# mcbuehler/Seg2Eye

Measured on AMD Instinct MI355X. Metric: images/sec per G+D train step, 256x256 bs=8, higher is better.
Workload: dtype bf16; 1 GPU; Seg2Eye G+D hinge-GAN train step (G step + D step, TTUR Adam, GAN + GAN_Feat), 256x256, batch 8 per GPU, ngf=ndf=64, 4 style images, synthetic ellipse labels, 4 batches in rotation; global_batch=8, parallelism=dp1, gradient_exchange=none, graph_segments_G=1

## Files before the change

### include/seg2eye_hip.h

```cpp
#ifndef SEG2EYE_HIP_H
#define SEG2EYE_HIP_H
#include <stddef.h>
#include <stdint.h>

#ifdef __cplusplus
extern "C" {
#endif

#define S2E_OK 0
#define S2E_ERR_ARG (-1)
#define S2E_ERR_LAUNCH (-2)
#define S2E_ERR_UNSUPPORTED (-3)

enum { S2E_F32 = 0, S2E_BF16 = 1 };
enum { S2E_ACT_NONE = 0, S2E_ACT_LRELU = 1, S2E_ACT_TANH = 2 };
enum { S2E_AUX_NONE = 0, S2E_AUX_RELU_MASK = 1, S2E_AUX_LRELU_GRAD = 2 };
enum { S2E_NORM_SPADE_STYLE = 0, S2E_NORM_PLAIN_IN = 1,
       S2E_NORM_SPADE_STYLE_BATCH = 2,
       S2E_NORM_ACCUMULATE_DX = 0x100 };
enum { S2E_LOSS_NEG_MEAN = 0, S2E_LOSS_HINGE_REAL = 1, S2E_LOSS_HINGE_FAKE = 2, S2E_LOSS_L1 = 3,
       S2E_LOSS_L1_NANGRAD = 4 };

int s2e_version(void);
const char* s2e_last_error(void);
// ... 126 lines not shown
    const int* rect_list; const int* rect_count;
    int N, H, W, Cin, Cout;
    int flags;
} s2e_wgrad_batch_job;
int s2e_wgrad_batch_supported(int dtype, int N, int H, int W, int Cin, int Cout);
size_t s2e_wgrad_batch_workspace_bytes(void);
int s2e_wgrad_batch(int dtype, const s2e_wgrad_batch_job* jobs, int n_jobs, void* workspace, size_t workspace_bytes, void* stream);
int s2e_spade_conv_modulate_rect(int dtype, int N, int H, int W, int C, int nh, int flags, int* tw, int* th);
#define S2E_UNI_REPLICAS 16
typedef struct s2e_spade_uni_job {
    const float* R; float* A; const float* w_gb; long w_sc, w_sk, w_st;
    const float* w_sh; const float* b_sh; float* dw_sh; float* db_sh; float* dw_gb; float* db_gb;
    int C2, nh, ncls, act_bf16;
} s2e_spade_uni_job;
int s2e_label_rect_lists_bwd(const uint8_t* cls, int N, int tiles_y, int tiles_x, int* work_list, int* ui_list, int* counts, void* stream);
int s2e_conv2d_rects_supported(int dtype, const s2e_conv_desc* d);
int s2e_conv2d_rects(int dtype, const void* x, const void* w_packed, const float* bias, const void* residual, const void* aux, void* y,
                     const s2e_conv_desc* d, const int* rect_list, const int* rect_count, void* stream);
size_t s2e_conv2d_wgrad_rects_workspace_bytes(int dtype, const s2e_conv_desc* d);
int s2e_conv2d_wgrad_rects(int dtype, const void* x, const void* gy, float* dw, float* dbias, const s2e_conv_desc* d,
                           const int* rect_list, const int* rect_count, void* workspace, size_t workspace_bytes, void* stream);
int s2e_spade_uniform_sums(int dtype, const void* dgb, int N, int H, int W, int C2, int ncls, const uint8_t* cls, const int* ui_list,
                           const int* counts, float* R, void* stream);
int s2e_spade_uniform_grads(const s2e_spade_uni_job* jobs_host, int n_jobs, void* stream);
int s2e_label_rect_classify(const uint8_t* label, int N, int H, int W, int h, int w, int tw, int th,
                            uint8_t* cls, int* dense_list, int* uni_list, int* counts, void* stream);
int s2e_spade_conv_modulate_sparse(int dtype, const void* actv, const void* w_packed, const float* bias, const void* x,
                                   const float* stats, const float* style, int style_ld, void* out, void* gamma_out,
                                   int N, int H, int W, int C, int nh, int lrelu, int flags, const int* dense_list,
                                   const int* counts, void* stream);
// ... 166 lines not shown
```

### seg2eye_amd/_lib.py

```python
import ctypes as C
import os

import torch

_HERE = os.path.dirname(os.path.abspath(__file__))
LIB_PATH = os.environ.get('S2E_LIB_PATH') or os.path.join(_HERE, 'lib', 'libseg2eye_hip.so')

S2E_F32, S2E_BF16 = 0, 1
UNI_REPLICAS = 16
SPADE_ANY_TILES, SPADE_DENSE, SPADE_ANY_RECTS, SPADE_X_HALF = 1, 2, 4, 8
ACT_NONE, ACT_LRELU, ACT_TANH = 0, 1, 2
AUX_NONE, AUX_RELU_MASK, AUX_LRELU_GRAD = 0, 1, 2
NORM_SPADE_STYLE, NORM_PLAIN_IN, NORM_SPADE_STYLE_BATCH = 0, 1, 2
NORM_ACCUMULATE_DX = 0x100
LOSS_NEG_MEAN, LOSS_HINGE_REAL, LOSS_HINGE_FAKE, LOSS_L1, LOSS_L1_NANGRAD = 0, 1, 2, 3, 4
REGION_L1, REGION_L2 = 0, 1
RANK_L2, RANK_MISMATCH = 0, 1


class ConvDesc(C.Structure):
    _fields_ = [(n, C.c_int) for n in (
        'N', 'Hi', 'Wi', 'Cin', 'Ho', 'Wo', 'Cout', 'KH', 'KW', 'stride', 'pad',
        'transposed', 'in_act', 'out_act', 'aux_mode')]

# ... 69 lines not shown
    's2e_weight_grads_batched': (STATUS, [_vp, _vp, _i, _i, _i, _vp, _vp]),
    's2e_unpack_weight_grad': (STATUS, [_vp, _vp, _i, _i, _i, _i, _i, _i, _vp]),
    's2e_pack_block_map': (COUNT, [_i, _vp, _i, _vp]),
    's2e_pack_conv_weights': (STATUS, [_i, _vp, _vp, _i, _i, _vp, _vp]),
    's2e_conv2d_workspace_bytes': (SIZE, [_i, C.POINTER(ConvDesc)]),
    's2e_conv2d_kernel_kind': (VALUE, [_i, C.POINTER(ConvDesc)]),
    's2e_conv2d_wgrad_kernel_kind': (VALUE, [_i, C.POINTER(ConvDesc)]),
    's2e_conv2d': (STATUS, [_i, _vp, _vp, _vp, _vp, _vp, _vp, C.POINTER(ConvDesc), _vp, C.c_size_t, _vp]),
    's2e_conv2d_plane_supported': (VALUE, [_i, C.POINTER(ConvDesc)]),
    's2e_conv_plane_weight_elems': (SIZE, [C.POINTER(ConvDesc)]),
    's2e_conv2d_plane': (STATUS, [_i, _vp, _vp, _vp, _vp, _vp, _vp, C.POINTER(ConvDesc), _vp]),
    's2e_conv2d_stats_slots': (VALUE, [_i, C.POINTER(ConvDesc)]),
    's2e_conv2d_stats': (STATUS, [_i, _vp, _vp, _vp, _vp, _vp, C.POINTER(ConvDesc), _vp, _vp]),
    's2e_in_stats_from_partials': (STATUS, [_vp, _i, _i, _i, _i, _f, _vp, _vp, _vp]),
    's2e_label_rect_lists_bwd': (STATUS, [_vp, _i, _i, _i, _vp, _vp, _vp, _vp]),
    's2e_conv2d_rects_supported': (VALUE, [_i, C.POINTER(ConvDesc)]),
    's2e_conv2d_rects': (STATUS, [_i, _vp, _vp, _vp, _vp, _vp, _vp, C.POINTER(ConvDesc), _vp, _vp, _vp]),
    's2e_conv2d_wgrad_rects_workspace_bytes': (SIZE, [_i, C.POINTER(ConvDesc)]),
    's2e_conv2d_wgrad_rects': (STATUS, [_i, _vp, _vp, _vp, _vp, C.POINTER(ConvDesc), _vp, _vp, _vp, C.c_size_t, _vp]),
    's2e_spade_uniform_sums': (STATUS, [_i, _vp, _i, _i, _i, _i, _i, _vp, _vp, _vp, _vp, _vp]),
    's2e_spade_uniform_grads': (STATUS, [_vp, _i, _vp]),
    's2e_conv2d_wgrad_workspace_bytes': (SIZE, [_i, C.POINTER(ConvDesc)]),
    's2e_conv2d_wgrad': (STATUS, [_i, _vp, _vp, _vp, _vp, C.POINTER(ConvDesc), _vp, C.c_size_t, _vp]),
    's2e_conv2d_wgrad_multi_supported': (VALUE, [_i, C.POINTER(ConvDesc)]),
    's2e_conv2d_wgrad_multi_kind': (VALUE, [_i, C.POINTER(ConvDesc)]),
    's2e_conv2d_wgrad_multi_workspace_bytes': (SIZE, [_i, _vp, _i]),
    's2e_conv2d_wgrad_multi': (STATUS, [_i, _vp, _i, _vp, C.c_size_t, _vp]),
    's2e_in_stats_workspace_bytes': (SIZE, [_i, _i, _i, _i]),
    's2e_modulate_bwd_workspace_bytes': (SIZE, [_i, _i, _i, _i]),
    's2e_instance_norm_fwd': (STATUS, [_i, _vp, _vp, _vp, _vp, _i, _i, _i, _f, _i, _vp]),
# ... 156 lines not shown
```

### seg2eye_amd/csrc/conv_duo.hip

```cpp
#include "conv_patch.h"
#include <stdlib.h>

namespace {

struct DuoParams {
    const void* x; const void* w; const float* bias; const void* res; const void* aux; void* y;
    int N, Hi, Wi, Cin, Ho, Wo, Cout, Kpad;
    int org, flip, out_act, aux_mode;
    int tw, th, sh, tw_shift;
    int tiles_x, tiles_y, tiles_n;
    int rects;
    unsigned x_bytes, w_bytes;
    const int* rect_list; const int* rect_count;
    const void* mx; const float* mstats; const float* mstyle; int msld; void* mgamma; int mC, mlrelu, mup;
    float* spart; int sP;
    long* dbg;
    int abl;
};

constexpr int DU_PPX = 400;
constexpr int DU_P_BYTES = DU_PPX * 64;
constexpr int DU_B_BYTES = 128 * 64;
constexpr int DU_NBS = 3, DU_PD = 2;

template <bool FUSE, int BN = 128, bool MF16 = false, int EPI = -1>
__global__ __launch_bounds__(256, 2) void conv_duo_kernel(const DuoParams p) {
    static_assert(BN == 128 || (BN == 64 && !FUSE), "tile widths");
    static_assert(!MF16 || BN == 128, "the 16x16x32 loop is written for 128-channel tiles");
    typedef bf16_t T;
    constexpr int NW = 4, TAPS = 9;
    constexpr int TM = BN / 32, TN = 2;
    constexpr int WROWS = TM * 32, NPASS = 2 * TM;
    constexpr int P_BYTES = DU_P_BYTES, B_BYTES = DU_B_BYTES, NBS = DU_NBS, PD = DU_PD;
    constexpr int NPIECE = P_BYTES / 1024;
    constexpr int NR = (NPIECE + NW - 1) / NW;
    constexpr int NBJ = BN / 64;
    constexpr int NR16 = 6;
    static_assert(NR <= TAPS, "one patch piece per tap must cover the patch");
    static_assert(NW * 4096 <= P_BYTES, "the waves' staging slices must fit one patch buffer");
    __shared__ __attribute__((aligned(16))) char smem[2 * P_BYTES + NBS * B_BYTES];
    __shared__ __attribute__((aligned(16))) float kcst[2][512];

// ... 160 lines not shown
        const int i = lane & 15, kq = lane >> 4;
#pragma unroll
        for (int dx = 0; dx < 3; ++dx)
            a16[dx] = lds0 + (uint32_t)(((8 * wm) * 18 + i + dx) * 64 + ((kq ^ (((i + dx) >> 1) & 3)) << 4));
        b16 = lds0 + 2 * P_BYTES + (uint32_t)((FUSE ? wn * 32 : wn * 64) * 64 + i * 64 + ((kq ^ ((i >> 1) & 3)) << 4));
    }
    auto read_al = [&](uint32_t ab, int dy) __attribute__((always_inline)) {
#pragma unroll
        for (int m = 0; m < 4; ++m)
            asm volatile("ds_read_b128 %0, %1 offset:%2" : "=v"(fal[m]) : "v"(ab), "n"((m + dy) * 1152) : "memory");
    };
    auto read_ah = [&](uint32_t ab, int dy) __attribute__((always_inline)) {
#pragma unroll
        for (int m = 0; m < 4; ++m)
            asm volatile("ds_read_b128 %0, %1 offset:%2" : "=v"(fah[m]) : "v"(ab), "n"((4 + m + dy) * 1152) : "memory");
    };
    auto read_b = [&](uint32_t bb, int par) __attribute__((always_inline)) {
#pragma unroll
        for (int n = 0; n < 4; ++n)
            asm volatile("ds_read_b128 %0, %1 offset:%2" : "=v"(fbb[par][n]) : "v"(bb), "n"(FUSE ? (n & 1) * 1024 + (n >> 1) * 4096 : n * 1024) : "memory");
    };
    auto mfma16 = [&](int half, int par) __attribute__((always_inline)) {
#pragma unroll
        for (int m = 0; m < 4; ++m)
#pragma unroll
            for (int n = 0; n < 4; ++n)
                acc16[MF16 ? half * 4 + m : 0][n] = __builtin_amdgcn_mfma_f32_16x16x32_bf16(
                    __builtin_bit_cast(bf16x8_t, half ? fah[m] : fal[m]), __builtin_bit_cast(bf16x8_t, fbb[par][n]), acc16[MF16 ? half * 4 + m : 0][n], 0, 0, 0);
    };

// ... 208 lines not shown
                }
            });
            *(u32x4_t*)(yg + so + lo) = u32x4_t{ov[0], ov[1], ov[2], ov[3]};
            if (gout) *(u32x4_t*)(gout + so + lo) = u32x4_t{gv[0], gv[1], gv[2], gv[3]};
        });
        st_issued = gout ? 16 : 8;
    };

    auto fetch_rect = [&](int id) __attribute__((always_inline)) -> int {
        if (p.rect_list && id < n_items) return p.rect_list[id / p.tiles_n];
        return -1;
    };

    Item cur = decode(item_id, fetch_rect(item_id));
    aim(cur);
    int pb = 0, cb = 0;
    prologue(cur, pb, cb);
    int tile_i = (int)blockIdx.x >= (G >> 1) ? 1 : 0;
#ifdef S2E_DUO_STAMPS
    int dbg_i = 0;
    const bool dbg_on = p.dbg && tid == 0 && ((int)blockIdx.x == 0 || (int)blockIdx.x == (G >> 1) || (int)blockIdx.x == 8);
    long* dbg_row = p.dbg ? p.dbg + ((int)blockIdx.x == 0 ? 0 : (int)blockIdx.x == 8 ? 2 : 1) * 64 : nullptr;
    auto stamp = [&](int k) __attribute__((always_inline)) { if (dbg_on && dbg_i < 12) dbg_row[dbg_i * 5 + k] = __builtin_amdgcn_s_memrealtime(); };
#else
    auto stamp = [&](int) __attribute__((always_inline)) {};
#endif
    for (;;) {
        stamp(0);
        if (st_issued >= 16) wait_vmcnt<16>();
        else if (st_issued >= 8) wait_vmcnt<8>();
// ... 43 lines not shown
                static_for<0, 2 * TAPS>([&](auto T) {
                    constexpr int t = decltype(T)::value;
                    constexpr int tap = t % TAPS, cc = t / TAPS, par = t & 1;
                    constexpr int ntap = (tap + 1) % TAPS, u = t + PD;
                    uint32_t pcb = cc ? pbs1 : pbs0, pnb = cc ? pbs0 : pbs1;
                    uint32_t nsb = (uint32_t)(((t + 1) % NBS) * B_BYTES);
                    int cs = c;
                    asm volatile("" : "+s"(pcb), "+s"(pnb), "+s"(nsb), "+s"(cs));
                    if (cs >= nch) return;
#ifdef S2E_DUO_STAMPS
                    const int abl = p.abl;
#else
                    constexpr int abl = 0;
#endif
                    if (!(abl & 1)) {
                        if constexpr (tap < NR16) { if (cc == 0 || !last) dma_patch16(tap, cs + cc + 1, pnb); }
                        if (u < 2 * TAPS || !last) dma_w16(cs + u / TAPS, u % TAPS, u % NBS);
                    }
                    if (!(abl & 4)) read_ah(a16[tap % 3] + pcb, tap / 3);
                    asm volatile("s_waitcnt lgkmcnt(4)" : "+v"(fal[0]), "+v"(fal[1]), "+v"(fal[2]), "+v"(fal[3]), "+v"(fbb[par][0]), "+v"(fbb[par][1]),
                                 "+v"(fbb[par][2]), "+v"(fbb[par][3]) :: "memory");
                    if (!(abl & 2)) mfma16(0, par);
                    constexpr int now_p = tap < NR16 ? 1 : 0, now_w = NBJ;
                    if constexpr (cc == 1 && (tap < NR16 || u >= 2 * TAPS)) {
                        if (last) wait_keep(u < 2 * TAPS ? now_w : 0); else wait_keep(now_p + now_w);
                    } else wait_keep(now_p + now_w);
                    asm volatile("s_waitcnt lgkmcnt(0)" : "+v"(fah[0]), "+v"(fah[1]), "+v"(fah[2]), "+v"(fah[3]) :: "memory");
                    if (!(abl & 8)) __builtin_amdgcn_s_barrier();
                    if (!(abl & 4)) {
                        if (t + 1 < 2 * TAPS || !last) {
                            read_al(a16[ntap % 3] + (ntap == 0 ? pnb : pcb), ntap / 3);
                            read_b(b16 + nsb, par ^ 1);
                        }
                    }
                    if (!(abl & 2)) mfma16(1, par);
                });
            }
        } else {
        float cinit[TN];
            {
// ... 12 lines not shown
            for (int mi = 0; mi < TM; ++mi)
    #pragma unroll
                for (int ni = 0; ni < TN; ++ni)
    #pragma unroll
                    for (int r = 0; r < 16; ++r) acc[mi][ni][r] = cinit[ni];
            int kt = 0, stage = 0;
            aim_frags(0, 0, pb, 0);
            read_frags(0, 0);
            for (int c = 0; c < nch; ++c) {
                const bool more = c + 1 < nch;
                const int pcur = (pb + c) & 1;
                static_for<0, TAPS>([&](auto TAP) {
                    constexpr int tap = decltype(TAP)::value;
                    constexpr int ntap = (tap + 1) % TAPS;
                    int issued = 0;
                    if constexpr (tap < NR) { if (more) issued += dma_patch(TAP, c + 1, pcur ^ 1); }
                    if (kt + PD < nk) { dma_w(kt + PD, stage == 0 ? NBS - 1 : stage - 1); issued += NBJ; }
                    read_frags(1, 1);
                    frags_ready(0, false);
                    mfmas(0);
                    wait_keep(issued);
                    frags_ready(1, true);
                    __builtin_amdgcn_s_barrier();
                    stage = stage == NBS - 1 ? 0 : stage + 1;
                    ++kt;
                    if (kt < nk) {
                        aim_frags(ntap / 3, ntap % 3, ntap == 0 ? pcur ^ 1 : pcur, stage);
                        read_frags(0, 0);
                    }
                    mfmas(1);
                });
            }
        }
        stamp(2);
        __builtin_amdgcn_s_setprio(0);
        const int pbn = (pb + nch) & 1;
        const int next_id = item_id + G;
        const bool has_next = next_id < n_items;
        Item nxt = cur;
        if constexpr (FUSE) load_mod_consts(cb);
        if (has_next) { nxt = decode(next_id, nf); aim(nxt); prologue(nxt, pbn, cb ^ 1); }
        stamp(3);
        if constexpr (FUSE) epilogue_fused(cur, pbn ^ 1);
        else if constexpr (EPI == 0) epilogue(cur, pbn ^ 1, std::integral_constant<int, 0>{}, std::false_type{});
        else if constexpr (EPI == 1) epilogue(cur, pbn ^ 1, std::integral_constant<int, 1>{}, std::false_type{});
        else if constexpr (EPI == 2) epilogue(cur, pbn ^ 1, std::integral_constant<int, 2>{}, std::false_type{});
// ... 8 lines not shown
        else epilogue(cur, pbn ^ 1, std::integral_constant<int, 0>{}, std::false_type{});
        stamp(4);
#ifdef S2E_DUO_STAMPS
        ++dbg_i;
#endif
        if (!has_next) break;
        cur = nxt; item_id = next_id; pb = pbn; cb ^= 1; ++tile_i;
    }
}

int duo_min_items() {
    static const int n = s2e_env_int("S2E_CONV_DUO", 256);
    return n;
}

template <bool FUSE>
int duo_launch(DuoParams& p, long rects_upper, hipStream_t st) {
    const long items = rects_upper * p.tiles_n;
    const int cap = 2 * s2e_cu_count();
    const int grid = items < cap ? (int)items : cap;
#ifdef S2E_DUO_STAMPS
    static long* const dbg_ptr = (long*)s2e_env_long("S2E_DUO_DBG_PTR", 0);
    p.dbg = dbg_ptr;
    static const int abl_env = s2e_env_int("S2E_DUO_ABL", 0);
    p.abl = abl_env;
#endif
    static const bool mf16 = s2e_env_flag("S2E_DUO_MF16", true);
    if (!FUSE && p.Cout <= 64) conv_duo_kernel<false, 64><<<grid, 256, 0, st>>>(p);
    else if (!mf16) conv_duo_kernel<FUSE><<<grid, 256, 0, st>>>(p);
    else if (FUSE) conv_duo_kernel<true, 128, true><<<grid, 256, 0, st>>>(p);
    else {
        const int epi = p.aux_mode != S2E_AUX_NONE ? 2 : (p.res ? 1 : 0) + (p.spart ? 3 : 0);
        if (epi == 0) conv_duo_kernel<false, 128, true, 0><<<grid, 256, 0, st>>>(p);
        else if (epi == 1) conv_duo_kernel<false, 128, true, 1><<<grid, 256, 0, st>>>(p);
        else if (epi == 2) conv_duo_kernel<false, 128, true, 2><<<grid, 256, 0, st>>>(p);
        else if (epi == 3) conv_duo_kernel<false, 128, true, 3><<<grid, 256, 0, st>>>(p);
        else conv_duo_kernel<false, 128, true, 4><<<grid, 256, 0, st>>>(p);
    }
    S2E_CHECK_LAUNCH("conv_duo_kernel");
    return S2E_OK;
}

}
// ... 36 lines not shown
int s2e_conv_duo_stats_slots(const s2e_conv_desc* d, const s2e_patch_plan* plan) {
    return (d->Ho / plan->th) * (d->Wo / plan->tw) * (d->Cout <= 64 ? 4 : 2);
}

int s2e_conv_duo_launch(const s2e_patch_plan* plan, const void* x, const void* w, const float* bias, const void* res,
                        const void* aux, void* y, const s2e_conv_desc* d, int kpad, float* stats_part, const int* rect_list,
                        const int* rect_count, hipStream_t st) {
    DuoParams p{};
    p.x = x; p.w = w; p.bias = bias; p.res = res; p.aux = aux; p.y = y;
    p.rect_list = rect_list; p.rect_count = rect_count;
    p.spart = stats_part; p.sP = stats_part ? s2e_conv_duo_stats_slots(d, plan) : 0;
    duo_fill(&p, d, plan, kpad);
    p.tiles_n = d->Cout <= 64 ? 1 : ceil_div(d->Cout, 128);
    p.w_bytes = (unsigned)((long)s2e_conv_cout_pad(d->Cout) * kpad * 2);
    return duo_launch<false>(p, p.rects, st);
}

int s2e_spade_conv_modulate_duo(int dtype, const void* actv, const void* w_packed, const float* bias, const void* x,
                                const float* stats, const float* style, int style_ld, void* out, void* gamma_out,
                                int N, int H, int W, int C, int nh, int lrelu, int flags, int tw, int th,
                                const int* rect_list, const int* rect_count, hipStream_t st) {
    if (duo_min_items() <= 0 || dtype != S2E_BF16 || nh % 32 != 0 || C % 64 != 0 || (flags & S2E_SPADE_ANY_TILES)) return 0;
    if (!duo_rect_ok(tw, th, H, W)) return 0;
    const long rects = (long)N * (H / th) * (W / tw);
    if (rects * (C / 64) < duo_min_items()) return 0;
    if ((long)N * H * W * nh * 2 >= (1L << 31) || (long)N * H * W * C * 2 >= (1L << 31)) return 0;
    const int kpad = ceil_div(9 * nh, 64) * 64;
    if ((long)s2e_conv_cout_pad(2 * C) * kpad * 2 >= (1L << 31)) return 0;
    const s2e_conv_desc d{N, H, W, nh, H, W, 2 * C, 3, 3, 1, 1, 0, S2E_ACT_NONE, S2E_ACT_NONE, S2E_AUX_NONE};
    const s2e_patch_plan plan{tw, th, 1, 0, 0};
// ... 12 lines not shown
```

### seg2eye_amd/csrc/conv_igemm.hip

```cpp
#include "common.h"
#include "conv_small.h"
#include "conv_patch.h"
#include "conv_stream.h"
#include <stdlib.h>

struct ConvKParams {
    const void* x; const void* w; const float* bias; const void* res; const void* aux; void* y;
    int N, Hi, Wi, Cin, Ho, Wo, Cout;
    int KH, KW, stride, pad, transposed;
    int in_act, out_act, aux_mode;
    int Ktot, Kpad, M, tiles_n;
    int tm_fast;
    int tiles, splits, kt_per_split;
    float* partial;
    int cls_tile0[5];
};


template <typename T, int BN, bool VECPATH, bool GLDS, bool S2 = false>
__global__ __launch_bounds__(256, 2) void conv_igemm_kernel(const ConvKParams p) {
    constexpr int BM = 128;
    constexpr int VEC = Vec<T>::N;
    constexpr int BK = 8 * VEC;
    constexpr int WN = (BN >= 64) ? 2 : 1;
// ... 550 lines not shown
extern "C" int s2e_conv2d_rects_supported(int dtype, const s2e_conv_desc* d) {
    return d && conv_route(dtype, d, false).kernel == ROUTE_DUO ? 1 : 0;
}

extern "C" int s2e_conv2d_rects(int dtype, const void* x, const void* w, const float* bias, const void* res, const void* aux, void* y,
                                const s2e_conv_desc* d, const int* rect_list, const int* rect_count, void* stream) {
    if (!x || !w || !y || !d || !rect_list || !rect_count) S2E_FAIL(S2E_ERR_ARG, "s2e_conv2d_rects: null pointer");
    if (d->aux_mode != S2E_AUX_NONE && !aux) S2E_FAIL(S2E_ERR_ARG, "s2e_conv2d_rects: aux_mode without aux");
    const ConvRoute r = conv_route(dtype, d, res && d->aux_mode != S2E_AUX_NONE);
    if (r.kernel != ROUTE_DUO)
        S2E_FAIL(S2E_ERR_UNSUPPORTED, "s2e_conv2d_rects: this shape's kernel takes no rectangle list (s2e_conv2d_rects_supported)");
    return s2e_conv_duo_launch(&r.patch, x, w, bias, res, aux, y, d, s2e_conv_k_pad(dtype, d->KH * d->KW * d->Cin), nullptr, rect_list, rect_count,
                               (hipStream_t)stream);
}

extern "C" int s2e_conv2d(int dtype, const void* x, const void* w, const float* bias, const void* res,
                          const void* aux, void* y, const s2e_conv_desc* d, void* workspace, size_t workspace_bytes,
                          void* stream) {
    if (!x || !w || !y || !d) S2E_FAIL(S2E_ERR_ARG, "s2e_conv2d: null pointer");
    if (d->stride != 1 && d->stride != 2) S2E_FAIL(S2E_ERR_UNSUPPORTED, "s2e_conv2d: stride %d", d->stride);
    if (d->N <= 0 || d->Cin <= 0 || d->Cout <= 0 || d->Ho <= 0 || d->Wo <= 0 || d->Hi <= 0 || d->Wi <= 0)
        S2E_FAIL(S2E_ERR_ARG, "s2e_conv2d: bad shape");
    if (d->aux_mode != S2E_AUX_NONE && !aux) S2E_FAIL(S2E_ERR_ARG, "s2e_conv2d: aux_mode without aux");
    if (d->KH * d->KW > 32) S2E_FAIL(S2E_ERR_UNSUPPORTED, "s2e_conv2d: kernel %dx%d has more than 32 taps", d->KH, d->KW);
    if ((long)d->N * d->Hi * d->Wi >= (1L << 31) || (long)d->N * d->Ho * d->Wo >= (1L << 31))
        S2E_FAIL(S2E_ERR_UNSUPPORTED, "s2e_conv2d: tensor too large for 32-bit pixel indices");
    const ConvRoute r = conv_route(dtype, d, res && d->aux_mode != S2E_AUX_NONE);
    if (r.workspace_bytes && (!workspace || workspace_bytes < r.workspace_bytes))
        S2E_FAIL(S2E_ERR_ARG, "s2e_conv2d: this shape needs %zu bytes of workspace (s2e_conv2d_workspace_bytes)", r.workspace_bytes);
    hipStream_t st = (hipStream_t)stream;
// ... 40 lines not shown
```

### seg2eye_amd/csrc/conv_patch.h

```cpp
#pragma once
#include "common.h"

struct s2e_patch_plan {
    int tw, th;
    int splits;
    int s2d;
    int bn;
};
int s2e_conv_patch_plan(int dtype, const s2e_conv_desc* d, s2e_patch_plan* plan);
int s2e_conv_patch_launch(int dtype, const s2e_patch_plan* plan, const void* x, const void* w, const float* bias, const void* res,
                          const void* aux, void* y, const s2e_conv_desc* d, int kpad, float* partial, hipStream_t st);

double s2e_patch_rectangle(const s2e_conv_desc* d, int ks, int* tw_out, int* th_out);

int s2e_conv_duo_plan(int dtype, const s2e_conv_desc* d, s2e_patch_plan* plan);
int s2e_conv_duo_launch(const s2e_patch_plan* plan, const void* x, const void* w, const float* bias, const void* res,
                        const void* aux, void* y, const s2e_conv_desc* d, int kpad, float* stats_part, const int* rect_list,
                        const int* rect_count, hipStream_t st);
int s2e_conv_duo_stats_slots(const s2e_conv_desc* d, const s2e_patch_plan* plan);
int s2e_spade_conv_modulate_duo(int dtype, const void* actv, const void* w_packed, const float* bias, const void* x,
                                const float* stats, const float* style, int style_ld, void* out, void* gamma_out,
                                int N, int H, int W, int C, int nh, int lrelu, int flags, int tw, int th,
                                const int* rect_list, const int* rect_count, hipStream_t st);
```

### seg2eye_amd/networks/architecture.py

```python
import torch
import torch.nn as nn
from torch.nn.utils import spectral_norm

from .. import ops
from ..spectral import sn_begin
from .normalization import SPADE_STYLE_Block, SegMap, spade_stats


class SPADE_STYLE_ResnetBlock(nn.Module):

    def __init__(self, fin, fout, opt):
        super().__init__()
        fmid = min(fin, fout)
        self.learned_shortcut = fin != fout
        wrap = spectral_norm if 'spectral' in opt.norm_G else (lambda conv: conv)
        convs = [('conv_0', fin, fmid, 3, True), ('conv_1', fmid, fout, 3, True)]
        norms = [('norm_0', fin), ('norm_1', fmid)]
        if self.learned_shortcut:
            convs.append(('conv_s', fin, fout, 1, False))
            norms.append(('norm_s', fin))
        for name, cin, cout, k, bias in convs:
            setattr(self, name, wrap(nn.Conv2d(cin, cout, kernel_size=k, padding=k // 2, bias=bias)))
        for name, c in norms:
            setattr(self, name, SPADE_STYLE_Block(c, opt))

    def input_stats(self, x, replication=1):
        ready = getattr(x, '_s2e_in_stats', None)
        if ready is not None and self.norm_0.spade.kind == 'instance':
            return ready
        return spade_stats(x, [self.norm_0.spade] + ([self.norm_s.spade] if self.learned_shortcut else []), replication)

    def _convs(self, h0, x_s, seg, latent_style):
        fused = self.norm_1.spade.kind == 'instance'
        s_dx, s_out = ([], []) if fused else (None, None)
        dx = ops.conv2d_m(h0, self.conv_0, None, 1, 1, stats_out=s_dx)
        out = ops.conv2d_m(self.norm_1(dx, seg, latent_style, s_dx[0] if s_dx else None, lrelu=True), self.conv_1, x_s, 1, 1, stats_out=s_out)
        if s_out:
            out._s2e_in_stats = s_out[0]
        return out

    def forward(self, x, seg, latent_style, stats=None, up=False):
        seg = SegMap.of(seg)
        sn_begin(self)
        fold = (up and self.learned_shortcut and stats is not None and self.norm_0.spade.kind != 'batch'
                and self.norm_0.takes_fold(x) and self.norm_s.takes_fold(x))
        if up and not fold:
            x = ops.upsample2x(x)
        if fold:
            if torch.is_grad_enabled() and x.requires_grad:
                h0, x = self.norm_0(x, seg, latent_style, stats, lrelu=True, relay=True, up=True)
            else:
                h0 = self.norm_0(x, seg, latent_style, stats, lrelu=True, up=True)
            x_s = ops.conv2d_m(self.norm_s(x, seg, latent_style, stats, lrelu=False, up=True), self.conv_s)
            return self._convs(h0, x_s, seg, latent_style)
        if stats is None:
            stats = self.input_stats(x)
        if torch.is_grad_enabled() and x.requires_grad:
            h0, x = self.norm_0(x, seg, latent_style, stats, lrelu=True, relay=True)
        else:
            h0 = self.norm_0(x, seg, latent_style, stats, lrelu=True)
        if self.learned_shortcut:
            x_s = ops.conv2d_m(self.norm_s(x, seg, latent_style, stats, lrelu=False), self.conv_s)
        else:
            x_s = x
        return self._convs(h0, x_s, seg, latent_style)
```

### seg2eye_amd/networks/generator.py

```python
import os

import torch
import torch.nn as nn

from .. import ops
from .._lib import ACT_LRELU, ACT_TANH
from ..options import latent_size
from .. import packing
from . import stylebank
from ..spectral import sn_begin
from .architecture import SPADE_STYLE_ResnetBlock
from .base_network import BaseNetwork, compute_dtype_of
from .normalization import SegMap


_FOLD_UP = os.environ.get('S2E_FOLD_UPSAMPLE', '1') != '0'


class SPADESTYLEGenerator(BaseNetwork):
    @staticmethod
    def modify_commandline_options(parser, is_train):
        parser.add_argument('--num_upsampling_layers', choices=('normal', 'more'), default='normal',
                            help="If 'more', adds upsampling layer between the two middle resnet blocks "
                                 "('most' is broken in the reference and not offered)")
# ... 1 lines not shown

    def __init__(self, opt):
        super().__init__()
        self.opt = opt
        self.cdtype = compute_dtype_of(opt)
        nf = opt.ngf
        self.sw, self.sh = latent_size(opt)
        self.fc = nn.Conv2d(opt.semantic_nc, 16 * nf, 3, padding=1)
        self.head_0 = SPADE_STYLE_ResnetBlock(16 * nf, 16 * nf, opt)
        self.G_middle_0 = SPADE_STYLE_ResnetBlock(16 * nf, 16 * nf, opt)
        self.G_middle_1 = SPADE_STYLE_ResnetBlock(16 * nf, 16 * nf, opt)
        self.up_0 = SPADE_STYLE_ResnetBlock(16 * nf, 8 * nf, opt)
        self.up_1 = SPADE_STYLE_ResnetBlock(8 * nf, 4 * nf, opt)
        self.up_2 = SPADE_STYLE_ResnetBlock(4 * nf, 2 * nf, opt)
        self.up_3 = SPADE_STYLE_ResnetBlock(2 * nf, 1 * nf, opt)
        self.conv_img = nn.Conv2d(nf, opt.output_nc, 3, padding=1)
        self.up = nn.Upsample(scale_factor=2)

    def forward(self, input, w=None):
        seg = SegMap.of(input)
        self.require_gpu(seg.label, w)
        n, H, W = seg.shape
        f = 32 if self.opt.num_upsampling_layers == 'normal' else 64
        if (H, W) != (self.sh * f, self.sw * f):
            raise ValueError('label map is %dx%d but this generator emits %dx%d (SURVEY F5)' % (H, W, self.sh * f, self.sw * f))
        w = w.float()
        bank = sn_begin(self)
        pre = self.__dict__.get('_spade_prepass')
        if pre is None:
            pre = self.__dict__['_spade_prepass'] = ops.SpadePrepass()
# ... 27 lines not shown
```

### seg2eye_amd/ops/conv.py

```python
import collections

import torch

from .. import _lib as L
from .. import packing
from .._lib import ConvDesc, ACT_NONE, ACT_LRELU, ACT_TANH, AUX_NONE, AUX_LRELU_GRAD
from .core import IN_EPS, LaunchProfiler, ZeroPool, _cl_dense, _cl_rows, _dt, _grad_dst, _need, _p, _stream, colsum, memo
from .sink import GradSink



PLANE_LAYOUT = 4


def pack_weight(w_oihw, dtype, cin_pad=None, transposed=False, sigma=None, plane=False):
    dt = _dt(dtype)
    w = w_oihw.detach()
    cout, cin, kh, kw = w.shape
    cin_pad = cin if cin_pad is None else cin_pad
    if plane:
        if dtype != torch.bfloat16 or cin_pad != cin:
            raise ValueError('pack_weight: the plane layout is bf16 without channel padding')
        cl = w.dtype == torch.float32 and not w.is_contiguous() and _cl_dense(w)
        if not cl and (w.dtype != torch.float32 or not w.is_contiguous()):
# ... 285 lines not shown
            gres = g
        return gx, gw, gb, gres, None, None, None, None, None, None, None, None


def conv2d(x, weight, bias=None, residual=None, stride=1, pad=0, in_act=ACT_NONE, out_act=ACT_NONE, sn=None, stats_out=None):
    u, v, sigma = sn if sn is not None else (None, None, None)
    return Conv2dFn.apply(x, weight, bias, residual, stride, pad, in_act, out_act, u, v, sigma, stats_out)


def conv2d_m(x, conv, residual=None, stride=1, pad=0, in_act=ACT_NONE, out_act=ACT_NONE, stats_out=None):
    from ..spectral import conv_params
    weight, bias, sn = conv_params(conv)
    return conv2d(x, weight, bias, residual, stride, pad, in_act, out_act, sn, stats_out)


class FcHeadFn(torch.autograd.Function):

    @staticmethod
    def forward(ctx, x, weight, bias, slope):
        _need(x, weight, bias)
        m, h, w, c = x.shape
        n = weight.shape[0]
        y = torch.empty(m, n, dtype=torch.float32, device=x.device)
        wsb = L.call.s2e_fc_head_fwd_workspace_bytes(m, h * w, c, n)
        ws = torch.empty(max(wsb // 4, 1), dtype=torch.float32, device=x.device)
        L.call.s2e_fc_head_fwd(_dt(x), _p(x), _p(weight), _p(bias), _p(y), m, h * w, c, n, float(slope), _p(ws), wsb, _stream())
        ctx.slope = float(slope)
        ctx.wdst, ctx.bdst = _grad_dst(weight), _grad_dst(bias)
        ctx.save_for_backward(x, weight)
        return y
# ... 21 lines not shown
```

### seg2eye_amd/ops/switches.py

```python
import os

_DET = os.environ.get('S2E_DETERMINISTIC', '0') == '1'

WGRAD_BATCH_OFF = os.environ.get('S2E_WGRAD_BATCH', '1') == '0' or _DET
WGRAD_MULTI_OFF = os.environ.get('S2E_WGRAD_MULTI', '1') == '0'
SPARSE_BWD_OFF = os.environ.get('S2E_SPADE_SPARSE_BWD', '1') == '0' or _DET
SPARSE_OFF = os.environ.get('S2E_SPADE_SPARSE', '1') == '0'
FUSED_OFF = os.environ.get('S2E_SPADE_FUSED', '1') == '0'
C8_SPARSE_OFF = os.environ.get('S2E_C8_SPARSE', '1') == '0'
```

Measured before the change: 539.5 images/s.

## Fold learned 1x1 shortcut conv into the 3x3 conv_1 duo kernel as extra K chunks

Adds a FOLD variant of the duo implicit-GEMM kernel that, after the 3x3 conv_1 accumulation, streams the shortcut activations and 1x1 weights through the patch and weight buffers as an extra K tail. The shortcut conv is then computed into the same accumulators instead of being materialised as a residual tensor. This is wired into the up_1..up_3 resnet blocks through a new autograd function whose backward calls the two existing conv backward paths. It saves one launch and the write and re-read of x_s per block, at the cost of more kernel template variants and a longer per-tile K loop.

```diff
diff --git a/include/seg2eye_hip.h b/include/seg2eye_hip.h
--- a/include/seg2eye_hip.h
+++ b/include/seg2eye_hip.h
@@ -164,6 +164,9 @@
     int C2, nh, ncls, act_bf16;
 } s2e_spade_uni_job;
 int s2e_label_rect_lists_bwd(const uint8_t* cls, int N, int tiles_y, int tiles_x, int* work_list, int* ui_list, int* counts, void* stream);
+int s2e_conv2d_fold1x1_supported(int dtype, const s2e_conv_desc* d, int Cin2);
+int s2e_conv2d_fold1x1(int dtype, const void* x, const void* w_packed, const float* bias, const void* x2, const void* w2_packed, void* y,
+                       const s2e_conv_desc* d, int Cin2, float* stats_part, void* stream);
 int s2e_conv2d_rects_supported(int dtype, const s2e_conv_desc* d);
 int s2e_conv2d_rects(int dtype, const void* x, const void* w_packed, const float* bias, const void* residual, const void* aux, void* y,
                      const s2e_conv_desc* d, const int* rect_list, const int* rect_count, void* stream);
diff --git a/seg2eye_amd/_lib.py b/seg2eye_amd/_lib.py
--- a/seg2eye_amd/_lib.py
+++ b/seg2eye_amd/_lib.py
@@ -107,6 +107,8 @@
     's2e_conv2d_stats': (STATUS, [_i, _vp, _vp, _vp, _vp, _vp, C.POINTER(ConvDesc), _vp, _vp]),
     's2e_in_stats_from_partials': (STATUS, [_vp, _i, _i, _i, _i, _f, _vp, _vp, _vp]),
     's2e_label_rect_lists_bwd': (STATUS, [_vp, _i, _i, _i, _vp, _vp, _vp, _vp]),
+    's2e_conv2d_fold1x1_supported': (VALUE, [_i, C.POINTER(ConvDesc), _i]),
+    's2e_conv2d_fold1x1': (STATUS, [_i, _vp, _vp, _vp, _vp, _vp, _vp, C.POINTER(ConvDesc), _i, _vp, _vp]),
     's2e_conv2d_rects_supported': (VALUE, [_i, C.POINTER(ConvDesc)]),
     's2e_conv2d_rects': (STATUS, [_i, _vp, _vp, _vp, _vp, _vp, _vp, C.POINTER(ConvDesc), _vp, _vp, _vp]),
     's2e_conv2d_wgrad_rects_workspace_bytes': (SIZE, [_i, C.POINTER(ConvDesc)]),
diff --git a/seg2eye_amd/csrc/conv_duo.hip b/seg2eye_amd/csrc/conv_duo.hip
--- a/seg2eye_amd/csrc/conv_duo.hip
+++ b/seg2eye_amd/csrc/conv_duo.hip
@@ -16,6 +16,7 @@
     float* spart; int sP;
     long* dbg;
     int abl;
+    const void* x2; const void* w2; int Cin2, Kpad2; unsigned x2_bytes, w2_bytes;
 };
 
 constexpr int DU_PPX = 400;
@@ -23,9 +24,10 @@
 constexpr int DU_B_BYTES = 128 * 64;
 constexpr int DU_NBS = 3, DU_PD = 2;
 
-template <bool FUSE, int BN = 128, bool MF16 = false, int EPI = -1>
+template <bool FUSE, int BN = 128, bool MF16 = false, int EPI = -1, bool FOLD = false>
 __global__ __launch_bounds__(256, 2) void conv_duo_kernel(const DuoParams p) {
     static_assert(BN == 128 || (BN == 64 && !FUSE), "tile widths");
+    static_assert(!FOLD || (!FUSE && (EPI == 0 || EPI == 3 || BN == 64)), "the fold is built for the plain epilogues of the up blocks");
     static_assert(!MF16 || BN == 128, "the 16x16x32 loop is written for 128-channel tiles");
     typedef bf16_t T;
     constexpr int NW = 4, TAPS = 9;
@@ -216,6 +218,16 @@
 #pragma unroll
         for (int m = 0; m < 4; ++m)
             asm volatile("ds_read_b128 %0, %1 offset:%2" : "=v"(fah[m]) : "v"(ab), "n"((4 + m + dy) * 1152) : "memory");
+    };
+    auto read_tl = [&](uint32_t ab) __attribute__((always_inline)) {
+#pragma unroll
+        for (int m = 0; m < 4; ++m)
+            asm volatile("ds_read_b128 %0, %1 offset:%2" : "=v"(fal[m]) : "v"(ab), "n"(m * 1024) : "memory");
+    };
+    auto read_th = [&](uint32_t ab) __attribute__((always_inline)) {
+#pragma unroll
+        for (int m = 0; m < 4; ++m)
+            asm volatile("ds_read_b128 %0, %1 offset:%2" : "=v"(fah[m]) : "v"(ab), "n"((4 + m) * 1024) : "memory");
     };
     auto read_b = [&](uint32_t bb, int par) __attribute__((always_inline)) {
 #pragma unroll
@@ -454,6 +466,28 @@
 
     Item cur = decode(item_id, fetch_rect(item_id));
     aim(cur);
+    constexpr int T_BYTES = 16 * 1024;
+    static_assert(3 * T_BYTES <= 2 * P_BYTES, "three tail chunks must fit the patch buffers");
+    auto fold_piece = [&](int r, int chunk, uint32_t tb) __attribute__((always_inline)) {
+        const __amdgpu_buffer_rsrc_t rx2 = __builtin_amdgcn_make_buffer_rsrc((void*)p.x2, 0, (int)p.x2_bytes, 0x00020000);
+        const int row = r * NW + wave, ltx = lane >> 2;
+        unsigned so = 2u * (unsigned)(((cur.n * p.Ho + cur.y0 + row) * p.Wo + cur.x0) * p.Cin2) + 64u * (unsigned)chunk;
+        asm volatile("" : "+s"(so));
+        const unsigned vo = 2u * (unsigned)(ltx * p.Cin2) + (unsigned)(((lane & 3) ^ ((ltx >> 1) & 3)) << 4);
+        __builtin_amdgcn_raw_ptr_buffer_load_lds(rx2, (lptr_t)(smem + tb + row * 1024), 16, (int)(vo + so), 0, 0, 0);
+    };
+    auto fold_w = [&](int chunk, int wstage) __attribute__((always_inline)) {
+        const __amdgpu_buffer_rsrc_t rw2 = __builtin_amdgcn_make_buffer_rsrc((void*)p.w2, 0, (int)p.w2_bytes, 0x00020000);
+        unsigned ko = 64u * (unsigned)chunk;
+        asm volatile("" : "+s"(ko));
+#pragma unroll
+        for (int j = 0; j < NBJ; ++j) {
+            const int trow = 16 * (wave + NW * j) + (lane >> 2);
+            const unsigned wo = 2u * (unsigned)((cur.tn * BN + trow) * p.Kpad2) + (unsigned)(((lane & 3) ^ ((MF16 ? trow >> 1 : trow >> 2) & 3)) << 4);
+            __builtin_amdgcn_raw_ptr_buffer_load_lds(rw2, (lptr_t)(smem + 2 * P_BYTES + wstage * B_BYTES + (wave + NW * j) * 1024), 16,
+                                                     (int)(wo + ko), 0, 0, 0);
+        }
+    };
     int pb = 0, cb = 0;
     prologue(cur, pb, cb);
     int tile_i = (int)blockIdx.x >= (G >> 1) ? 1 : 0;
@@ -527,8 +561,12 @@
                     constexpr int abl = 0;
 #endif
                     if (!(abl & 1)) {
-                        if constexpr (tap < NR16) { if (cc == 0 || !last) dma_patch16(tap, cs + cc + 1, pnb); }
+                        if constexpr (tap < NR16) {
+                            if (cc == 0 || !last) dma_patch16(tap, cs + cc + 1, pnb);
+                            else if constexpr (FOLD && tap < 4) fold_piece(tap, 0, pb ? 2 * T_BYTES : 0);
+                        }
                         if (u < 2 * TAPS || !last) dma_w16(cs + u / TAPS, u % TAPS, u % NBS);
+                        else if constexpr (FOLD) fold_w(u - 2 * TAPS, u % NBS);
                     }
                     if (!(abl & 4)) read_ah(a16[tap % 3] + pcb, tap / 3);
                     asm volatile("s_waitcnt lgkmcnt(4)" : "+v"(fal[0]), "+v"(fal[1]), "+v"(fal[2]), "+v"(fal[3]), "+v"(fbb[par][0]), "+v"(fbb[par][1]),
@@ -536,7 +574,7 @@
                     if (!(abl & 2)) mfma16(0, par);
                     constexpr int now_p = tap < NR16 ? 1 : 0, now_w = NBJ;
                     if constexpr (cc == 1 && (tap < NR16 || u >= 2 * TAPS)) {
-                        if (last) wait_keep(u < 2 * TAPS ? now_w : 0); else wait_keep(now_p + now_w);
+                        if (last) wait_keep(FOLD ? (tap < 4 ? 1 : 0) + now_w : (u < 2 * TAPS ? now_w : 0)); else wait_keep(now_p + now_w);
                     } else wait_keep(now_p + now_w);
                     asm volatile("s_waitcnt lgkmcnt(0)" : "+v"(fah[0]), "+v"(fah[1]), "+v"(fah[2]), "+v"(fah[3]) :: "memory");
                     if (!(abl & 8)) __builtin_amdgcn_s_barrier();
@@ -579,8 +617,12 @@
                     constexpr int tap = decltype(TAP)::value;
                     constexpr int ntap = (tap + 1) % TAPS;
                     int issued = 0;
-                    if constexpr (tap < NR) { if (more) issued += dma_patch(TAP, c + 1, pcur ^ 1); }
+                    if constexpr (tap < NR) {
+                        if (more) issued += dma_patch(TAP, c + 1, pcur ^ 1);
+                        else if constexpr (FOLD && tap < 4) { fold_piece(tap, 0, pb ? 2 * T_BYTES : 0); issued += 1; }
+                    }
                     if (kt + PD < nk) { dma_w(kt + PD, stage == 0 ? NBS - 1 : stage - 1); issued += NBJ; }
+                    else if constexpr (FOLD) { fold_w(kt + PD - nk, stage == 0 ? NBS - 1 : stage - 1); issued += NBJ; }
                     read_frags(1, 1);
                     frags_ready(0, false);
                     mfmas(0);
@@ -595,6 +637,82 @@
                     }
                     mfmas(1);
                 });
+            }
+        }
+        if constexpr (FOLD) {
+            constexpr int LPS = 4 + NBJ;
+            const int nch2 = p.Cin2 >> 5;
+            int ps = pb ? 2 : 0, wsg = 0;
+            auto next3 = [](int v) __attribute__((always_inline)) { return v == 2 ? 0 : v + 1; };
+            auto dma_tail = [&](int chunk, int pst, int wst) __attribute__((always_inline)) {
+#pragma unroll
+                for (int r = 0; r < 4; ++r) fold_piece(r, chunk, (uint32_t)(pst * T_BYTES));
+                fold_w(chunk, wst);
+            };
+#pragma unroll
+            for (int r = 0; r < 4; ++r) fold_piece(r, 1, (uint32_t)(next3(ps) * T_BYTES));
+            if constexpr (MF16) {
+                const int i = lane & 15, kq = lane >> 4;
+                const uint32_t a16c = lds0 + (uint32_t)(((8 * wm) * 16 + i) * 64 + ((kq ^ ((i >> 1) & 3)) << 4));
+                read_tl(a16c + (uint32_t)(ps * T_BYTES));
+                read_b(b16, 0);
+                for (int j = 0; j < nch2; j += 2) {
+                    static_for<0, 2>([&](auto U) {
+                        constexpr int par = decltype(U)::value;
+                        int jj = j + par;
+                        asm volatile("" : "+s"(jj));
+                        const bool more2 = jj + 2 < nch2, more1 = jj + 1 < nch2;
+                        const int pn = next3(ps), wn2 = next3(wsg);
+                        if (more2) dma_tail(jj + 2, next3(pn), next3(wn2));
+                        read_th(a16c + (uint32_t)(ps * T_BYTES));
+                        asm volatile("s_waitcnt lgkmcnt(4)" : "+v"(fal[0]), "+v"(fal[1]), "+v"(fal[2]), "+v"(fal[3]), "+v"(fbb[par][0]), "+v"(fbb[par][1]),
+                                     "+v"(fbb[par][2]), "+v"(fbb[par][3]) :: "memory");
+                        mfma16(0, par);
+                        if (more2) wait_vmcnt<LPS>(); else wait_vmcnt<0>();
+                        asm volatile("s_waitcnt lgkmcnt(0)" : "+v"(fah[0]), "+v"(fah[1]), "+v"(fah[2]), "+v"(fah[3]) :: "memory");
+                        __builtin_amdgcn_s_barrier();
+                        if (more1) {
+                            read_tl(a16c + (uint32_t)(pn * T_BYTES));
+                            read_b(b16 + (uint32_t)(wn2 * B_BYTES), par ^ 1);
+                        }
+                        mfma16(1, par);
+                        ps = pn; wsg = wn2;
+                    });
+                }
+            } else {
+                uint32_t a_c[TM];
+#pragma unroll
+                for (int mi = 0; mi < TM; ++mi) {
+                    const int r = wm * WROWS + mi * 32 + l31;
+                    a_c[mi] = lds0 + (uint32_t)(r * 64 + ((h ^ (((r & 15) >> 1) & 3)) << 4));
+                }
+                auto aim_tail = [&](int pst, int wst) __attribute__((always_inline)) {
+                    int ua = pst * T_BYTES;
+                    asm volatile("" : "+s"(ua));
+#pragma unroll
+                    for (int mi = 0; mi < TM; ++mi) a_addr[mi] = a_c[mi] + (uint32_t)ua;
+#pragma unroll
+                    for (int ni = 0; ni < TN; ++ni) b_addr[ni] = b_off[ni] + wst * B_BYTES;
+                };
+                aim_tail(ps, 0);
+                read_frags(0, 0);
+                for (int j = 0; j < nch2; ++j) {
+                    const bool more2 = j + 2 < nch2, more1 = j + 1 < nch2;
+                    const int pn = next3(ps), wn2 = next3(wsg);
+                    if (more2) dma_tail(j + 2, next3(pn), next3(wn2));
+                    read_frags(1, 1);
+                    frags_ready(0, false);
+                    mfmas(0);
+                    if (more2) wait_vmcnt<LPS>(); else wait_vmcnt<0>();
+                    frags_ready(1, true);
+                    __builtin_amdgcn_s_barrier();
+                    ps = pn; wsg = wn2;
+                    if (more1) {
+                        aim_tail(ps, wsg);
+                        read_frags(0, 0);
+                    }
+                    mfmas(1);
+                }
             }
         }
         stamp(2);
@@ -633,7 +751,7 @@
     return n;
 }
 
-template <bool FUSE>
+template <bool FUSE, bool FOLD = false>
 int duo_launch(DuoParams& p, long rects_upper, hipStream_t st) {
     const long items = rects_upper * p.tiles_n;
     const int cap = 2 * s2e_cu_count();
@@ -645,7 +763,14 @@
     p.abl = abl_env;
 #endif
     static const bool mf16 = s2e_env_flag("S2E_DUO_MF16", true);
-    if (!FUSE && p.Cout <= 64) conv_duo_kernel<false, 64><<<grid, 256, 0, st>>>(p);
+    if constexpr (FOLD) {
+        if (p.Cout <= 64) conv_duo_kernel<false, 64, false, -1, true><<<grid, 256, 0, st>>>(p);
+        else if (!mf16 && p.spart) conv_duo_kernel<false, 128, false, 3, true><<<grid, 256, 0, st>>>(p);
+        else if (!mf16) conv_duo_kernel<false, 128, false, 0, true><<<grid, 256, 0, st>>>(p);
+        else if (p.spart) conv_duo_kernel<false, 128, true, 3, true><<<grid, 256, 0, st>>>(p);
+        else conv_duo_kernel<false, 128, true, 0, true><<<grid, 256, 0, st>>>(p);
+    }
+    else if (!FUSE && p.Cout <= 64) conv_duo_kernel<false, 64><<<grid, 256, 0, st>>>(p);
     else if (!mf16) conv_duo_kernel<FUSE><<<grid, 256, 0, st>>>(p);
     else if (FUSE) conv_duo_kernel<true, 128, true><<<grid, 256, 0, st>>>(p);
     else {
@@ -712,6 +837,27 @@
     p.tiles_n = d->Cout <= 64 ? 1 : ceil_div(d->Cout, 128);
     p.w_bytes = (unsigned)((long)s2e_conv_cout_pad(d->Cout) * kpad * 2);
     return duo_launch<false>(p, p.rects, st);
+}
+
+int s2e_conv_duo_fold_ok(int dtype, const s2e_conv_desc* d, int Cin2, s2e_patch_plan* plan) {
+    if (d->transposed || d->pad != 1 || d->aux_mode != S2E_AUX_NONE || Cin2 <= 0 || Cin2 % 64 != 0) return 0;
+    if (!s2e_conv_duo_plan(dtype, d, plan)) return 0;
+    if ((long)d->N * d->Ho * d->Wo * Cin2 * 2 >= (1L << 31)) return 0;
+    return (long)s2e_conv_cout_pad(d->Cout) * s2e_conv_k_pad(dtype, Cin2) * 2 < (1L << 31);
+}
+
+int s2e_conv_duo_launch_fold(const s2e_patch_plan* plan, const void* x, const void* w, const float* bias, const void* x2,
+                             const void* w2, void* y, const s2e_conv_desc* d, int kpad, int Cin2, float* stats_part, hipStream_t st) {
+    DuoParams p{};
+    p.x = x; p.w = w; p.bias = bias; p.y = y;
+    p.spart = stats_part; p.sP = stats_part ? s2e_conv_duo_stats_slots(d, plan) : 0;
+    duo_fill(&p, d, plan, kpad);
+    p.tiles_n = d->Cout <= 64 ? 1 : ceil_div(d->Cout, 128);
+    p.w_bytes = (unsigned)((long)s2e_conv_cout_pad(d->Cout) * kpad * 2);
+    p.x2 = x2; p.w2 = w2; p.Cin2 = Cin2; p.Kpad2 = s2e_conv_k_pad(S2E_BF16, Cin2);
+    p.x2_bytes = (unsigned)((long)d->N * d->Ho * d->Wo * Cin2 * 2);
+    p.w2_bytes = (unsigned)((long)s2e_conv_cout_pad(d->Cout) * p.Kpad2 * 2);
+    return duo_launch<false, true>(p, p.rects, st);
 }
 
 int s2e_spade_conv_modulate_duo(int dtype, const void* actv, const void* w_packed, const float* bias, const void* x,
diff --git a/seg2eye_amd/csrc/conv_igemm.hip b/seg2eye_amd/csrc/conv_igemm.hip
--- a/seg2eye_amd/csrc/conv_igemm.hip
+++ b/seg2eye_amd/csrc/conv_igemm.hip
@@ -588,6 +588,25 @@
                                (hipStream_t)stream);
 }
 
+static bool fold1x1_route(int dtype, const s2e_conv_desc* d, int Cin2, s2e_patch_plan* plan) {
+    if (!d || d->KH != 3 || d->KW != 3 || d->N <= 0 || d->Cin <= 0 || d->Cout <= 0 || d->Hi <= 0 || d->Wi <= 0) return false;
+    return conv_route(dtype, d, false).kernel == ROUTE_DUO && s2e_conv_duo_fold_ok(dtype, d, Cin2, plan);
+}
+
+extern "C" int s2e_conv2d_fold1x1_supported(int dtype, const s2e_conv_desc* d, int Cin2) {
+    s2e_patch_plan plan;
+    return fold1x1_route(dtype, d, Cin2, &plan) ? 1 : 0;
+}
+
+extern "C" int s2e_conv2d_fold1x1(int dtype, const void* x, const void* w, const float* bias, const void* x2, const void* w2, void* y,
+                                  const s2e_conv_desc* d, int Cin2, float* stats_part, void* stream) {
+    if (!x || !w || !x2 || !w2 || !y || !d) S2E_FAIL(S2E_ERR_ARG, "s2e_conv2d_fold1x1: null pointer");
+    s2e_patch_plan plan;
+    if (!fold1x1_route(dtype, d, Cin2, &plan))
+        S2E_FAIL(S2E_ERR_UNSUPPORTED, "s2e_conv2d_fold1x1: not a shape of the folded launch (s2e_conv2d_fold1x1_supported)");
+    return s2e_conv_duo_launch_fold(&plan, x, w, bias, x2, w2, y, d, s2e_conv_k_pad(dtype, 9 * d->Cin), Cin2, stats_part, (hipStream_t)stream);
+}
+
 extern "C" int s2e_conv2d(int dtype, const void* x, const void* w, const float* bias, const void* res,
                           const void* aux, void* y, const s2e_conv_desc* d, void* workspace, size_t workspace_bytes,
                           void* stream) {
diff --git a/seg2eye_amd/csrc/conv_patch.h b/seg2eye_amd/csrc/conv_patch.h
--- a/seg2eye_amd/csrc/conv_patch.h
+++ b/seg2eye_amd/csrc/conv_patch.h
@@ -18,6 +18,9 @@
                         const void* aux, void* y, const s2e_conv_desc* d, int kpad, float* stats_part, const int* rect_list,
                         const int* rect_count, hipStream_t st);
 int s2e_conv_duo_stats_slots(const s2e_conv_desc* d, const s2e_patch_plan* plan);
+int s2e_conv_duo_fold_ok(int dtype, const s2e_conv_desc* d, int Cin2, s2e_patch_plan* plan);
+int s2e_conv_duo_launch_fold(const s2e_patch_plan* plan, const void* x, const void* w, const float* bias, const void* x2,
+                             const void* w2, void* y, const s2e_conv_desc* d, int kpad, int Cin2, float* stats_part, hipStream_t st);
 int s2e_spade_conv_modulate_duo(int dtype, const void* actv, const void* w_packed, const float* bias, const void* x,
                                 const float* stats, const float* style, int style_ld, void* out, void* gamma_out,
                                 int N, int H, int W, int C, int nh, int lrelu, int flags, int tw, int th,
diff --git a/seg2eye_amd/networks/architecture.py b/seg2eye_amd/networks/architecture.py
--- a/seg2eye_amd/networks/architecture.py
+++ b/seg2eye_amd/networks/architecture.py
@@ -13,6 +13,7 @@
         super().__init__()
         fmid = min(fin, fout)
         self.learned_shortcut = fin != fout
+        self.shortcut_fold_mask = 7
         wrap = spectral_norm if 'spectral' in opt.norm_G else (lambda conv: conv)
         convs = [('conv_0', fin, fmid, 3, True), ('conv_1', fmid, fout, 3, True)]
         norms = [('norm_0', fin), ('norm_1', fmid)]
@@ -30,11 +31,22 @@
             return ready
         return spade_stats(x, [self.norm_0.spade] + ([self.norm_s.spade] if self.learned_shortcut else []), replication)
 
-    def _convs(self, h0, x_s, seg, latent_style):
+    def _shortcut(self, h0, s):
+        n, h, w, _ = h0.shape
+        if ops.shortcut_fold_ready(h0.dtype, n, h, w, self.conv_1.in_channels, self.conv_1.out_channels, self.conv_s.in_channels,
+                                   self.shortcut_fold_mask):
+            return s, True
+        return ops.conv2d_m(s, self.conv_s), False
+
+    def _convs(self, h0, x_s, seg, latent_style, fold_s=False):
         fused = self.norm_1.spade.kind == 'instance'
         s_dx, s_out = ([], []) if fused else (None, None)
         dx = ops.conv2d_m(h0, self.conv_0, None, 1, 1, stats_out=s_dx)
-        out = ops.conv2d_m(self.norm_1(dx, seg, latent_style, s_dx[0] if s_dx else None, lrelu=True), self.conv_1, x_s, 1, 1, stats_out=s_out)
+        h1 = self.norm_1(dx, seg, latent_style, s_dx[0] if s_dx else None, lrelu=True)
+        if fold_s:
+            out = ops.conv2d_shortcut_m(h1, self.conv_1, x_s, self.conv_s, stats_out=s_out, mask=self.shortcut_fold_mask)
+        else:
+            out = ops.conv2d_m(h1, self.conv_1, x_s, 1, 1, stats_out=s_out)
         if s_out:
             out._s2e_in_stats = s_out[0]
         return out
@@ -51,16 +63,17 @@
                 h0, x = self.norm_0(x, seg, latent_style, stats, lrelu=True, relay=True, up=True)
             else:
                 h0 = self.norm_0(x, seg, latent_style, stats, lrelu=True, up=True)
-            x_s = ops.conv2d_m(self.norm_s(x, seg, latent_style, stats, lrelu=False, up=True), self.conv_s)
-            return self._convs(h0, x_s, seg, latent_style)
+            x_s, fold_s = self._shortcut(h0, self.norm_s(x, seg, latent_style, stats, lrelu=False, up=True))
+            return self._convs(h0, x_s, seg, latent_style, fold_s)
         if stats is None:
             stats = self.input_stats(x)
         if torch.is_grad_enabled() and x.requires_grad:
             h0, x = self.norm_0(x, seg, latent_style, stats, lrelu=True, relay=True)
         else:
             h0 = self.norm_0(x, seg, latent_style, stats, lrelu=True)
+        fold_s = False
         if self.learned_shortcut:
-            x_s = ops.conv2d_m(self.norm_s(x, seg, latent_style, stats, lrelu=False), self.conv_s)
+            x_s, fold_s = self._shortcut(h0, self.norm_s(x, seg, latent_style, stats, lrelu=False))
         else:
             x_s = x
-        return self._convs(h0, x_s, seg, latent_style)
+        return self._convs(h0, x_s, seg, latent_style, fold_s)
diff --git a/seg2eye_amd/networks/generator.py b/seg2eye_amd/networks/generator.py
--- a/seg2eye_amd/networks/generator.py
+++ b/seg2eye_amd/networks/generator.py
@@ -39,6 +39,9 @@
         self.up_1 = SPADE_STYLE_ResnetBlock(8 * nf, 4 * nf, opt)
         self.up_2 = SPADE_STYLE_ResnetBlock(4 * nf, 2 * nf, opt)
         self.up_3 = SPADE_STYLE_ResnetBlock(2 * nf, 1 * nf, opt)
+        for bit, blk in enumerate((self.up_1, self.up_2, self.up_3)):
+            blk.shortcut_fold_mask = 1 << bit
+        self.up_0.shortcut_fold_mask = 0
         self.conv_img = nn.Conv2d(nf, opt.output_nc, 3, padding=1)
         self.up = nn.Upsample(scale_factor=2)
 
diff --git a/seg2eye_amd/ops/conv.py b/seg2eye_amd/ops/conv.py
--- a/seg2eye_amd/ops/conv.py
+++ b/seg2eye_amd/ops/conv.py
@@ -323,6 +323,86 @@
     return conv2d(x, weight, bias, residual, stride, pad, in_act, out_act, sn, stats_out)
 
 
+def shortcut_fold_ready(dtype, n, h, w, cmid, cout, cin2, mask=7):
+    from . import switches
+    if not (switches.SHORTCUT_FOLD & mask) or dtype != torch.bfloat16:
+        return False
+    shape = (n, h, w, cmid, h, w, cout, 3, 3, 1, 1, 0, ACT_NONE, ACT_NONE, AUX_NONE)
+    if _conv_shape(False, L.S2E_BF16, *shape).plane:
+        return False
+    return memo('fold1x1', shape + (cin2,), lambda: bool(L.call.s2e_conv2d_fold1x1_supported(L.S2E_BF16, ConvDesc(*shape), cin2)))
+
+
+class _BackwardCtx:
+
+    def __init__(self, saved, cfg, live, wdst, bdst, plan, plan_gen, needs):
+        self.saved_tensors, self.cfg, self.live, self.wdst, self.bdst = saved, cfg, live, wdst, bdst
+        self.plan, self.plan_gen, self.needs_input_grad = plan, plan_gen, needs
+
+
+class ShortcutFoldFn(torch.autograd.Function):
+
+    @staticmethod
+    def forward(ctx, h, w1, b1, s, ws, u1, v1, sigma1, us, vs, sigmas, stats_out=None):
+        n, hh, ww, cmid = h.shape
+        cout, cin2 = ws.shape[0], ws.shape[1]
+        if w1.shape[1] != cmid or s.shape != (n, hh, ww, cin2) or w1.shape[0] != cout:
+            raise ValueError('ShortcutFoldFn: shapes of the two convs do not meet')
+        plan = packing.current()
+        wp1 = packed_weight(w1, h.dtype, cmid, False, sigma1, plan)
+        wp2 = packed_weight(ws, h.dtype, cin2, False, sigmas, plan)
+        b = None if b1 is None else b1.detach().float().contiguous()
+        _need(h, s, wp1, wp2, b)
+        dt = _dt(h)
+        d, _, _, slots, _ = _conv_shape(False, dt, n, hh, ww, cmid, hh, ww, cout, 3, 3, 1, 1, 0, ACT_NONE, ACT_NONE, AUX_NONE)
+        y = torch.empty(n, hh, ww, cout, dtype=h.dtype, device=h.device)
+        part = torch.empty(n * slots * cout * 2, dtype=torch.float32, device=h.device) if (stats_out is not None and slots) else None
+        LaunchProfiler.run(
+            'conv_patch', 2.0 * n * hh * ww * cout * (9 * cmid + cin2),
+            L.call.s2e_conv2d_fold1x1, (dt, _p(h), _p(wp1), _p(b), _p(s), _p(wp2), _p(y), d, cin2, _p(part), _stream()),
+            tag=lambda: 'F n%d %dx%d c%d->%d k3 s1 +1x1 c%d%s' % (n, hh, ww, cmid, cout, cin2, ' +stats' if part is not None else ''),
+            nbytes=lambda: float((h.numel() + s.numel() + y.numel() + wp1.numel() + wp2.numel()) * h.element_size()))
+        if part is not None:
+            wsum = torch.empty(n * cout * 2, dtype=torch.float64, device=h.device)
+            stats = torch.empty(n, cout, 2, dtype=torch.float32, device=h.device)
+            LaunchProfiler.run('in_stats', 0.0, L.call.s2e_in_stats_from_partials,
+                               (_p(part), n, slots, cout, hh * ww, IN_EPS, _p(wsum), _p(stats), _stream()), nbytes=float(part.numel() * 4))
+            stats_out.append(stats)
+        ctx.plan, ctx.plan_gen = plan, (plan.generation if plan is not None else None)
+        ctx.live = LivePrefix.n
+        ctx.has_bias = b1 is not None
+        ctx.dst = (_grad_dst(w1), _grad_dst(b1) if b1 is not None else None, _grad_dst(ws))
+        ctx.save_for_backward(h, w1, u1, v1, sigma1, s, ws, us, vs, sigmas)
+        return y
+
+    @staticmethod
+    def backward(ctx, gy):
+        h, w1, u1, v1, sigma1, s, ws, us, vs, sigmas = ctx.saved_tensors
+        need = ctx.needs_input_grad
+        wdst1, bdst1, wdsts = ctx.dst
+        g = gy.contiguous()
+        c1 = _BackwardCtx((h, w1, None, u1, v1, sigma1), (1, 1, ACT_NONE, ACT_NONE, ctx.has_bias, False), ctx.live, wdst1, bdst1,
+                          ctx.plan, ctx.plan_gen, (need[0], need[1], need[2], False))
+        cs = _BackwardCtx((s, ws, None, us, vs, sigmas), (1, 0, ACT_NONE, ACT_NONE, False, False), ctx.live, wdsts, None,
+                          ctx.plan, ctx.plan_gen, (need[3], need[4], False, False))
+        gh, gw1, gb1 = Conv2dFn.backward(c1, g)[:3]
+        gs, gws = Conv2dFn.backward(cs, g)[:2]
+        return gh, gw1, gb1, gs, gws, None, None, None, None, None, None, None
+
+
+def conv2d_shortcut_m(h, conv_1, s, conv_s, stats_out=None, mask=7):
+    from ..spectral import conv_params
+    w1, b1, sn1 = conv_params(conv_1)
+    ws, bs, sns = conv_params(conv_s)
+    n, hh, ww, cmid = h.shape
+    if (bs is None and tuple(ws.shape[2:]) == (1, 1) and tuple(w1.shape[2:]) == (3, 3) and s.shape[:3] == h.shape[:3] and s.dtype == h.dtype
+            and w1.shape[1] == cmid and ws.shape[1] == s.shape[3]
+            and shortcut_fold_ready(h.dtype, n, hh, ww, cmid, w1.shape[0], ws.shape[1], mask)):
+        return ShortcutFoldFn.apply(h, w1, b1, s, ws, *(sn1 if sn1 is not None else (None, None, None)),
+                                    *(sns if sns is not None else (None, None, None)), stats_out)
+    return conv2d(h, w1, b1, conv2d(s, ws, bs, None, 1, 0, ACT_NONE, ACT_NONE, sns), 1, 1, ACT_NONE, ACT_NONE, sn1, stats_out)
+
+
 class FcHeadFn(torch.autograd.Function):
 
     @staticmethod
diff --git a/seg2eye_amd/ops/switches.py b/seg2eye_amd/ops/switches.py
--- a/seg2eye_amd/ops/switches.py
+++ b/seg2eye_amd/ops/switches.py
@@ -8,3 +8,4 @@
 SPARSE_OFF = os.environ.get('S2E_SPADE_SPARSE', '1') == '0'
 FUSED_OFF = os.environ.get('S2E_SPADE_FUSED', '1') == '0'
 C8_SPARSE_OFF = os.environ.get('S2E_C8_SPARSE', '1') == '0'
+SHORTCUT_FOLD = int(os.environ.get('S2E_SHORTCUT_FOLD', '7')) & 7
```

Result: no change. 544.3 images/s (median of 6 runs) (+0.9%).
